# AntreasAntoniou/HowToTrainYourMAMLPytorch

Measured on NVIDIA H100. Metric: meta-tasks/sec (5-way, 5 inner steps, second order), higher is better.
Workload: dtype fp32

## Files before the change

howtotrainyourmamlpytorch_b200/csrc/common.cuh:

```cuda
#pragma once
#include <cuda_runtime.h>
#include <stdint.h>
#include <string>

#define MAML_MAX_LAYERS 4
#define MAML_MAX_STEPS 8
#define BN_EPS_D 1e-5
#define LEAKY_SLOPE_F 0.01f

struct LayerGeom {
  int h, w;
  int cin;
  int gw, G;
  int ph, pw;
  int pgw, pG, pb;
  int guard;
};

struct ConvSrc {
  const float* A; long long a_stride;
  const float* W; long long w_stride;
  int kc;
  int wt;
  int sign;
};

enum { CONV_PLAIN = 0, CONV_FWD_STATS = 1, CONV_TAN_STATS = 2 };

struct ConvArgs {
  ConvSrc src[2]; int nsrc;
  const float* bias; long long bias_stride;
  float* out; long long out_stride;
  int rows;
  int gw, G, h, w;
  int ncols;
  int mode;
  const float* zh; long long zh_stride;
  double* stats; long long stats_stride;
  int tasks;
  double alg_flops;
  int tag;
};

struct Conv0Args {
  const float* X; long long x_stride;
  const float* W; long long w_stride;
  const float* bias; long long bias_stride;
  float* out; long long out_stride;
  int rows, gw, G, h, w, c0, ncols, mode;
  const float* zh; long long zh_stride;
  double* stats; long long stats_stride;
  int tasks;
  double alg_flops;
  int tag;
};

struct WgradArgs {
  const float* A[2]; long long a_stride[2];
  const float* D[2]; long long d_stride[2];
  long long a_plane[2], d_plane[2];
  int nsrc;
  int kc, ncols, rows, gw;
  int rows_per_chunk, nchunks;
  float* partial; long long partial_task_stride; long long chunk_stride;
  int tasks;
  double alg_flops;
  int tag;
};

struct InputGradArgs {
  const float* D[2]; long long d_stride[2];
  const float* W[2]; long long w_stride;
  float* dx; long long dx_stride;
  int nsrc;
  int rows, gw, G, h, w, c0, ncols;
  int tasks;
  double alg_flops;
  int tag;
};

struct BnGeom { int n, h, w, gw, G, ph, pw, pgw, pG, pb, F; };

struct BnActArgs {
  float* z; long long z_stride;
  const double* stats; long long stats_stride;
  const float* gamma; const float* beta;
  float* p; long long p_stride;
  float* p_hi; float* p_lo;
  BnGeom g; int tasks;
  int tag;
};

struct BnActTanArgs {
  float* zdot; long long zdot_stride;
  const float* zdot2;
  const float* zh; long long zh_stride;
  const double* stats_fwd; long long stats_fwd_stride;
  const double* stats_tan; long long stats_tan_stride;
  const float* gamma; const float* beta;
  float* pdot; long long pdot_stride;
  float* pdot_hi; float* pdot_lo;
  BnGeom g; int tasks;
  int tag;
};

struct BnBwdArgs {
  const float* dp; long long dp_stride;
  const float* zh; long long zh_stride;
  const double* stats_fwd; long long stats_fwd_stride;
  double* stats_bwd; long long stats_bwd_stride;
  const float* gamma; const float* beta;
  float* dz; long long dz_stride;
  float* dz_hi; float* dz_lo;
  BnGeom g; int tasks;
  int tag;
};

struct BnBwdTanArgs {
  const float* dp; long long dp_stride;
  const float* dpdot; long long dpdot_stride;
  const float* dpdot2;
  const float* zh; long long zh_stride;
  const float* zhdot; long long zhdot_stride;
  const float* dz; long long dz_stride;
  const double* stats_fwd; long long stats_fwd_stride;
  const double* stats_bwd; long long stats_bwd_stride;
  const double* stats_tan; long long stats_tan_stride;
  double* stats_tbwd; long long stats_tbwd_stride;
  const float* gamma; const float* beta;
  float* dzdot; long long dzdot_stride;
  float* dzdot_hi; float* dzdot_lo;
  BnGeom g; int tasks;
  int tag;
};

struct LnArgs {
  float* z; long long z_stride;
  const float* z2;
  const float* zh; long long zh_stride;
  const float* zhd; long long zhd_stride;
  const float* dp; long long dp_stride;
  const float* dpd; const float* dpd2; long long dpd_stride;
  const float* dz; long long dz_stride;
  float* out; float* out_hi; float* out_lo; long long out_stride;
  const double* st_fwd;
  const double* st_tan;
  const double* st_bwd;
  double* st_out;
// ... 75 lines not shown
void launch_bnbwd_tan(const BnBwdTanArgs& a, cudaStream_t st);
void launch_bnact_ibn(const BnActArgs& a, long long gb_stride, cudaStream_t st);
void launch_bnbwd_ibn(const BnBwdArgs& a, long long gb_stride, cudaStream_t st);
void launch_bnact_tan_ibn(const BnActTanArgs& a, long long gb_stride, const float* gdot, const float* bdot, cudaStream_t st);
void launch_bnbwd_tan_ibn(const BnBwdTanArgs& a, long long gb_stride, const float* gdot, cudaStream_t st);
void launch_ln_stats(const LnArgs& a, bool tan, cudaStream_t st);
void launch_ln_act(const LnArgs& a, bool tan, cudaStream_t st);
void launch_ln_bwd(const LnArgs& a, bool tan, cudaStream_t st);
void launch_ln_bias_grad(const LnArgs& a, bool tan, cudaStream_t st);
bool tail_fusable(const BnGeom& g, int n_rows, int rows_per_cta);
void launch_tail_fused(const BnActArgs& fa, const HeadArgs& ha, const BnBwdArgs& ba, cudaStream_t st);
void launch_tail_tan_fused(const BnActTanArgs& fa, const HeadArgs& ha, const BnBwdTanArgs& ba, cudaStream_t st);
void launch_head(const HeadArgs& a, cudaStream_t st);

void launch_import_theta(const ParamLayout& pl, const float* meta, float* theta0, long long theta_task_stride,
                         int tasks, cudaStream_t st, long long meta_task_stride = 0);
void launch_param_reduce(const ParamLayout& pl, const PartialDesc& pd, const float* partial, int mode,
                         const float* theta_in, float* theta_out, float* g_out, float* tbar,
                         const float* meta, int step, long long task_stride, int tasks, cudaStream_t st,
                         int seg_lo = 0, int seg_hi = -1);
void launch_dots_u(const ParamLayout& pl, float* tbar, const float* tgrad, const float* g, float* u, double* abar,
                   const float* meta, int step, long long task_stride, int tasks, cudaStream_t st);

#define MAML_MAX_RANKS 8
struct CommDev {
  int rank, world;
  float* local_data; long long slot_stride;
  unsigned* local_flags;
  unsigned* seq;
  unsigned* counters;
  const float* peer_data[MAML_MAX_RANKS];
  unsigned* peer_flags[MAML_MAX_RANKS];
  long long* status;
};

struct ExportArgs {
  CommDev comm;
  ParamLayout pl;
  const float* tbar; long long task_stride;
  const double* abar;
  const double* stats; long long stats_task_stride;
  long long st_pass_stride, st_layer_stride;
  const float* losses;
  const float* correct;
  float weights[MAML_MAX_STEPS];
  unsigned target_mask; int num_steps; int training;
  int tasks, task_offset, tasks_global;
  int n_s, n_t;
  int hw[MAML_MAX_LAYERS];
  float* result;
  int per_task; long long result_stride;
  const float* lnb;
  int tag;
};
void launch_export(const ExportArgs& a, cudaStream_t st);
void launch_allreduce(const CommDev& c, float* result, long long n, cudaStream_t st);
void launch_publish(const CommDev& c, const float* src, long long n, cudaStream_t st);

void launch_adam(float* meta, const float* grad, float* m, float* v, long long n, float lr, float bc1, float bc2,
                 const long long* seg_end_host, int nseg, unsigned trainable_mask, unsigned clamp_mask,
                 cudaStream_t st);
void launch_running_update(const float* part_mean, const float* part_var, float* rm, float* rv,
                           const float* decay_dev, int L, int S, int F, cudaStream_t st);
void launch_running_ema_from_stats(const double* stats, long long stats_task_stride, long long layer_stride, int tasks, float* rm,
                                   float* rv, int L, int S, int F, int step, const int* hw_host, int n, cudaStream_t st);

void launch_episode_gather(const float* dataset, const long long* image_index, const int* rot_k, int B, int N, int K, int T, int C,
                           int H, int W, const float* mean, const float* stdv, float* xs, float* xt, long long* ys, long long* yt,
                           cudaStream_t st);

enum { PASS_SUP_FWD = 0, PASS_SUP_BWD = 1, PASS_TGT_FWD = 2, PASS_TGT_BWD = 3, PASS_TAN_FWD = 4, PASS_TAN_BWD = 5,
       PASS_KINDS = 6 };

struct EngineOptions {
  bool no_graph = false;
  bool one_stream = false;
  bool wgrad_tc = true;
  int tc_split = 8;
  int tc_nb = 0;
  bool bn_fuse = true;
  bool tail_fuse = true;
  int tail_onchip = 3;
  int pdl = -1;
  int tc_timeline = -1;
  std::string graph_dot;
};

struct Profiler;
struct LaunchContext {
  const EngineOptions* opt;
  bool pdl;
  cudaStream_t main_stream;
  Profiler* prof;
};
const LaunchContext& launch_ctx();

inline bool pdl_allowed(cudaStream_t st) {
  const LaunchContext& c = launch_ctx();
  return c.pdl && st == c.main_stream;
}
int num_sms();

#define MAML_TRACE_ARMED 0x40000000
static __device__ unsigned long long* t_trace_buf = nullptr;
#define MAML_TRACE_SETTER(fn) void fn(unsigned long long* p) { cudaMemcpyToSymbol(t_trace_buf, &p, sizeof(p)); }
#define MAML_TRACE_CAP 4094
__device__ __forceinline__ void trace_mark(int kid, int tag = 0) {
  if (!(tag & MAML_TRACE_ARMED)) return;
  unsigned long long* t = t_trace_buf;
  if (t != nullptr && threadIdx.x == 0 && blockIdx.x == 0 && blockIdx.y == 0 && blockIdx.z == 0) {
    unsigned long long now;
    asm volatile("mov.u64 %0, %%globaltimer;" : "=l"(now));
    const unsigned long long slot = atomicAdd(t, 1ULL);
    if (slot < MAML_TRACE_CAP) t[1 + slot] = (now << 20) | ((unsigned long long)(tag & 0xfff) << 8) | (unsigned long long)(kid & 0xff);
  }
}
void trace_set_conv(unsigned long long* p);
void trace_set_bn(unsigned long long* p);
void trace_set_head(unsigned long long* p);
void trace_set_param(unsigned long long* p);
void trace_set_tc(unsigned long long* p);

__device__ __forceinline__ void pdl_prologue(int kid = 0, int tag = 0) {
  trace_mark(kid, tag);
  asm volatile("griddepcontrol.launch_dependents;" ::: "memory");
  asm volatile("griddepcontrol.wait;" ::: "memory");
}
__device__ __forceinline__ void pdl_trigger() { asm volatile("griddepcontrol.launch_dependents;" ::: "memory"); }
__device__ __forceinline__ void pdl_wait() { asm volatile("griddepcontrol.wait;" ::: "memory"); }
template <typename... KArgs, typename... Args>
inline void launch_pdl(void (*kernel)(KArgs...), dim3 grid, dim3 block, size_t smem, cudaStream_t st, Args&&... args) {
  cudaLaunchConfig_t cfg{};
  cfg.gridDim = grid; cfg.blockDim = block; cfg.dynamicSmemBytes = smem; cfg.stream = st;
  cudaLaunchAttribute attr[1];
  attr[0].id = cudaLaunchAttributeProgrammaticStreamSerialization;
  attr[0].val.programmaticStreamSerializationAllowed = pdl_allowed(st) ? 1 : 0;
  cfg.attrs = attr; cfg.numAttrs = 1;
  cudaLaunchKernelEx(&cfg, kernel, static_cast<KArgs>(args)...);
}

extern long long g_launch_counter;
extern long long g_launch_base;
extern int g_trace_flag;
inline int launch_tag() { return (int)(g_launch_counter - g_launch_base) | g_trace_flag; }
template <class A> inline A tagged(const A& a) { A t = a; t.tag = launch_tag(); return t; }

#define CUDA_CHECK_LAUNCH() do { g_launch_counter++; } while (0)

enum { PROF_CONV = 0, PROF_CONV0 = 1, PROF_WGRAD = 2, PROF_WGRAD0 = 3, PROF_BN = 4, PROF_HEAD = 5, PROF_PARAM = 6,
       PROF_CATS = 7 };
void prof_begin(Profiler* p, int cat, double flops, cudaStream_t st);
void prof_end(Profiler* p, cudaStream_t st);
struct ProfScope {
  cudaStream_t st; Profiler* prof;
  ProfScope(int cat, double flops, cudaStream_t s) : st(s), prof(launch_ctx().prof) { if (prof) prof_begin(prof, cat, flops, st); }
  ~ProfScope() { if (prof) prof_end(prof, st); }
};
```

howtotrainyourmamlpytorch_b200/csrc/engine.cu:

```cuda
#include <cstdio>
#include <cstdlib>
#include <cstring>
#include <cmath>
#include <string>
#include <vector>

#include "../../include/maml_b200.h"
#include "common.cuh"
#include "tc_common.cuh"

static thread_local std::string g_err;
static int fail(const std::string& m) { g_err = m; return 1; }

#define CK(call) do { cudaError_t e__ = (call); if (e__ != cudaSuccess) { \
  return fail(std::string(#call) + ": " + cudaGetErrorString(e__)); } } while (0)

static inline long long rup(long long x, long long m) { return (x + m - 1) / m * m; }

struct Profiler {
  struct Rec { int cat; double flops; cudaEvent_t a, b; };
  std::vector<Rec> recs;
  std::vector<cudaEvent_t> pool;
  size_t used = 0;
  cudaEvent_t get() {
    if (used == pool.size()) { cudaEvent_t e; cudaEventCreate(&e); pool.push_back(e); }
    return pool[used++];
  }
  void reset() { recs.clear(); used = 0; }
  ~Profiler() { for (auto e : pool) cudaEventDestroy(e); }
};
void prof_begin(Profiler* p, int cat, double flops, cudaStream_t st) {
  Profiler::Rec r; r.cat = cat; r.flops = flops; r.a = p->get(); r.b = p->get();
  cudaEventRecord(r.a, st);
  p->recs.push_back(r);
}
void prof_end(Profiler* p, cudaStream_t st) { cudaEventRecord(p->recs.back().b, st); }

static EngineOptions read_options() {
  auto flag = [](const char* name, bool def) { const char* v = getenv(name); return v ? atoi(v) != 0 : def; };
  auto num = [](const char* name, int def) { const char* v = getenv(name); return v ? atoi(v) : def; };
  auto clamp = [](int v, int lo, int hi) { return std::max(lo, std::min(hi, v)); };
  EngineOptions o;
  o.no_graph = getenv("MAML_B200_NO_GRAPH") != nullptr;
  o.one_stream = getenv("MAML_B200_ONE_STREAM") != nullptr;
  o.wgrad_tc = flag("MAML_B200_WGRAD_TC", o.wgrad_tc);
  o.tc_split = clamp(num("MAML_B200_TC_SPLIT", o.tc_split), 1, 8);
  if (getenv("MAML_B200_TC_NB")) o.tc_nb = clamp(num("MAML_B200_TC_NB", 0), 2, 8);
  o.bn_fuse = flag("MAML_B200_BN_FUSE", o.bn_fuse);
  o.tail_fuse = flag("MAML_B200_TAIL_FUSE", o.tail_fuse);
  o.tail_onchip = num("MAML_B200_TAIL_ONCHIP", o.tail_onchip);
  if (const char* v = getenv("MAML_B200_PDL")) o.pdl = atoi(v) != 0 ? 1 : 0;
  if (getenv("MAML_B200_TC_TIMELINE")) o.tc_timeline = std::max(0, num("MAML_B200_TC_TIMELINE", 0));
  if (const char* v = getenv("MAML_B200_GRAPH_DOT")) o.graph_dot = v;
  return o;
}

struct PassSet {
  int n = 0, slots = 0;
  float* xg = nullptr; long long xg_stride = 0;
  float* ain[MAML_MAX_LAYERS + 1] = {}; long long ain_sz[MAML_MAX_LAYERS + 1] = {};
  float* zh[MAML_MAX_LAYERS] = {}; long long zh_sz[MAML_MAX_LAYERS] = {};
  float* dz[MAML_MAX_LAYERS] = {}; long long dz_sz[MAML_MAX_LAYERS] = {};
  float* dp[MAML_MAX_LAYERS] = {}; long long dp_sz[MAML_MAX_LAYERS] = {};
  float* ain_base[MAML_MAX_LAYERS + 1] = {}; long long ain_plane[MAML_MAX_LAYERS + 1] = {};
  float* dz_base[MAML_MAX_LAYERS] = {}; long long dz_plane[MAML_MAX_LAYERS] = {};
  CUtensorMap ain_map[MAML_MAX_LAYERS][2];
  CUtensorMap dz_map[MAML_MAX_LAYERS][2];
};

struct ChunkPlan { int rows_per_chunk[MAML_MAX_LAYERS]; int nchunks[MAML_MAX_LAYERS]; PartialDesc pd; long long size; int head_groups; };
static inline int head_rows(int n) { return n <= 16 ? 16 : 4; }

struct maml_b200_handle {
  maml_b200_config cfg;
  EngineOptions opt;
  int L, F, N, S, C, H, W, n_s, n_t, maxT, D, pix;
  LayerGeom geo[MAML_MAX_LAYERS];
  ParamLayout pl;
  long long Ppad;
  std::vector<long long> seg_off, seg_size;
  char* ws = nullptr; long long ws_bytes = 0;
  PassSet sup, tgt, tan, tan2;
  float *theta = nullptr, *g = nullptr, *tgrad = nullptr, *tbar = nullptr, *u = nullptr;
  float *sup_partial = nullptr, *tgt_partial = nullptr;
  ChunkPlan plan_sup, plan_tgt;
  double* stats = nullptr; long long stats_task_stride = 0, st_pass_stride = 0, st_layer_stride = 0, stats_count = 0;
  float *losses = nullptr, *correct = nullptr, *decay_dev = nullptr;
  double* abar = nullptr;
  bool ln = false;
  double* ln_stats = nullptr; long long ln_task_stride = 0, ln_pass_stride = 0;
  float* lnb = nullptr;
  long long* zero_labels = nullptr;
  float* pinned = nullptr;
  int pin_slot = 0;
  long long last_launches = 0;
  int last_tasks = 0;
  int fn_kind = 0, fn_tasks = 0, fn_step = 0;
  float* xdot_g = nullptr;
  float* zero_dl = nullptr;
  Profiler prof;
  bool profiling = false;
  cudaStream_t s_cap = nullptr, s_tgt = nullptr, s_tgt2 = nullptr, s_wg = nullptr;
  int tgt_slots = 1;
  cudaEvent_t ev_fork = nullptr, ev_wg = nullptr, ev_pack = nullptr, ev_tgt[MAML_MAX_STEPS] = {};
  cudaEvent_t ev_pre[2 * MAML_MAX_LAYERS] = {};
  bool use_graphs = true;
  bool pdl = false;
  int nb_main = 8;
  bool wg_pending = false;
  struct GraphEntry { maml_b200_iter_args it; const void* p[7]; cudaGraphExec_t exec; long long launches; unsigned long long stamp; };
  std::vector<GraphEntry> graphs;
  unsigned long long graph_clock = 0;
  bool use_tc = false;
  float *pack_theta = nullptr, *pack_u = nullptr;
  long long pack_theta_plane = 0, pack_u_plane = 0, pack_task = 0;
  CUtensorMap theta_map[4], u_map[4];
  CommDev comm{};
  char* comm_block = nullptr; long long comm_bytes = 0;
  void* comm_opened[MAML_MAX_RANKS] = {};
  bool comm_connected = false;
};

enum { FN_NONE = 0, FN_FORWARD = 1, FN_BACKWARD = 2, FN_HVP = 4 };
static void record_call(maml_b200_handle* h, int kind, int n_tasks, int num_step) {
  h->fn_kind = kind; h->fn_tasks = n_tasks; h->fn_step = num_step;
}
static std::string call_names(int kinds) {
  std::string s;
  for (int k : {FN_FORWARD, FN_BACKWARD, FN_HVP})
    if (kinds & k)
      s += std::string(s.empty() ? "" : " or ") + (k == FN_FORWARD ? "maml_b200_net_forward" : k == FN_BACKWARD ? "maml_b200_net_backward" : "maml_b200_net_hvp");
  return s;
}
static int require_call(const maml_b200_handle* h, int kinds, int n_tasks, int num_step, const char* entry) {
// ... 466 lines not shown
  cudaEventRecord(h->ev_wg, h->s_wg);
  h->wg_pending = true;
}

static void reduce_lower(maml_b200_handle* h, const ReduceSpec& rs, const PartialDesc& pd, const float* partial,
                         const float* meta, int T, cudaStream_t st) {
  launch_param_reduce(h->pl, with_bn_sums(h, pd, rs.bn_sums), partial, rs.mode, rs.theta_in, rs.theta_out, rs.g_out, rs.tbar,
                      meta, rs.step, h->Ppad, T, st, 0, seg_per_block(h->pl));
}
static void join_pending(maml_b200_handle* h, cudaStream_t st) {
  if (!h->wg_pending) return;
  cudaStreamWaitEvent(st, h->ev_wg, 0);
  h->wg_pending = false;
}

static void tc_conv(maml_b200_handle* h, int l, int n, const TcOp& op, const float* bias, long long bias_stride,
                    float* out, long long out_stride, int mode, const float* zh, long long zh_stride, double* stats, int T,
                    cudaStream_t st) {
  const LayerGeom& g = h->geo[l];
  TcMaps maps;
  TcConvArgs a{};
  a.kc = h->F; a.rows = n * g.G; a.gw = g.gw; a.G = g.G; a.h = g.h; a.w = g.w; a.ncols = h->F; a.mode = mode; a.tasks = T; a.plan_tasks = h->maxT;
  a.halo = g.gw + 1; a.rpad = tc_conv_rpad(g.gw); a.nb = std::min(tc_conv_ring(h->F, g.gw), h->nb_main);
  a.timeline = (h->opt.tc_timeline == 0 || h->opt.tc_timeline == l) ? 1 : 0;
  maps.m[0] = op.a_maps[0]; maps.m[1] = op.a_maps[1];
  maps.m[2] = op.b_maps[op.b_pair]; maps.m[3] = op.b_maps[op.b_pair + 1];
  a.a_row_base = op.a_row_base; a.a_task_rows = op.a_task_rows; a.sign = op.sign;
  a.b_row_base = op.b_row_base; a.b_task_rows = op.b_task_rows;
  a.bias = bias; a.bias_stride = bias_stride; a.out = out; a.out_stride = out_stride;
  a.zh = zh; a.zh_stride = zh_stride; a.stats = stats; a.stats_stride = h->stats_task_stride;
  a.alg_flops = conv_flops(h, l, n, T, 1);
  launch_conv_tc(maps, a, st);
}

struct FfmaOp { const float* A; long long a_stride; const float* wv; int wt, sign; };

static ConvArgs ffma_conv(const maml_b200_handle* h, int l, int n, int mode, std::initializer_list<FfmaOp> ops,
                          const float* bias_vec, int T) {
  const LayerGeom& g = h->geo[l];
  ConvArgs a{};
  for (const FfmaOp& o : ops) a.src[a.nsrc++] = ConvSrc{o.A, o.a_stride, o.wv + h->pl.w_off[l], h->Ppad, h->F, o.wt, o.sign};
  if (bias_vec) { a.bias = bias_vec + h->pl.b_off[l]; a.bias_stride = h->Ppad; }
  a.rows = n * g.G; a.gw = g.gw; a.G = g.G; a.h = g.h; a.w = g.w; a.ncols = h->F; a.mode = mode;
  if (mode != CONV_PLAIN) a.stats_stride = h->stats_task_stride;
  a.tasks = T;
  a.alg_flops = conv_flops(h, l, n, T, a.nsrc);
  return a;
}

static Conv0Args conv0_args(const maml_b200_handle* h, const PassSet& ps, const float* wv, int mode, int nsrc, int T) {
  const LayerGeom& g = h->geo[0];
  Conv0Args a{};
  a.X = ps.xg; a.x_stride = ps.xg_stride;
  a.W = wv + h->pl.w_off[0]; a.w_stride = h->Ppad;
  a.bias = wv + h->pl.b_off[0]; a.bias_stride = h->Ppad;
  a.rows = ps.n * g.G; a.gw = g.gw; a.G = g.G; a.h = g.h; a.w = g.w; a.c0 = h->C; a.ncols = h->F; a.mode = mode;
  a.stats_stride = h->stats_task_stride; a.tasks = T;
  a.alg_flops = conv_flops(h, 0, ps.n, T, nsrc);
  return a;
}

static WgradArgs wgrad_args(const maml_b200_handle* h, int l, int n, const ChunkPlan& cp, float* partial, int T) {
  const LayerGeom& g = h->geo[l];
  WgradArgs w{};
  w.kc = l == 0 ? h->C : h->F; w.ncols = h->F; w.rows = n * g.G; w.gw = g.gw;
  w.rows_per_chunk = cp.rows_per_chunk[l]; w.nchunks = cp.nchunks[l];
  const int k = seg_per_block(h->pl) * l;
  w.partial = partial + cp.pd.off[k]; w.partial_task_stride = cp.pd.task_stride; w.chunk_stride = cp.pd.cstride[k];
  w.tasks = T;
  return w;
}

struct WgPair { Slot a, d; };

static void launch_wgrad_upper(const maml_b200_handle* h, int l, int n, const ChunkPlan& cp, float* partial, int T,
                               std::initializer_list<WgPair> pairs, cudaStream_t st) {
  const bool tc = h->use_tc && h->opt.wgrad_tc;
  WgradArgs w = wgrad_args(h, l, n, cp, partial, T);
  for (const WgPair& p : pairs) {
    const PassSet& pa = *p.a.ps; const PassSet& pd = *p.d.ps;
    const int k = w.nsrc++;
    w.A[k] = AIN(pa, l, p.a.slot); w.a_stride[k] = STRIDE(pa, ain, l);
    w.D[k] = DZ(pd, l, p.d.slot); w.d_stride[k] = STRIDE(pd, dz, l);
    if (tc) { w.a_plane[k] = pa.ain_plane[l]; w.d_plane[k] = pd.dz_plane[l]; }
  }
  w.alg_flops = conv_flops(h, l, n, T, w.nsrc);
  if (tc) launch_wgrad_tc(w, st);
  else launch_wgrad(w, st);
}

static HeadArgs head_args(const maml_b200_handle* h, int mode, const PassSet& ps, int slot, const float* theta, int T) {
  HeadArgs a{};
  a.mode = mode; a.n = ps.n; a.N = h->N; a.D = h->D; a.scale = 1.f;
  a.f = AIN(ps, h->L, slot); a.f_stride = STRIDE(ps, ain, h->L);
  a.Wfc = theta + h->pl.fcw_off; a.bfc = theta + h->pl.fcb_off; a.theta_stride = h->Ppad;
  a.y = h->zero_labels; a.y_stride = 0;
  a.rows_per_cta = head_rows(ps.n);
  if (mode != HEAD_TARGET_FWD) { a.df = DP(ps, h->L - 1, slot); a.df_stride = STRIDE(ps, dp, h->L - 1); }
  a.tasks = T;
  return a;
}

static void head_grad(const maml_b200_handle* h, HeadArgs& a, float* partial, const ChunkPlan& cp) {
  const int k = seg_per_block(h->pl) * h->L;
  a.gW = partial + cp.pd.off[k]; a.gb = partial + cp.pd.off[k + 1];
  a.g_stride = cp.pd.task_stride; a.g_chunk_stride = cp.pd.cstride[k];
}

static bool support_tail_fused(const maml_b200_handle* h) {
  return h->opt.tail_fuse && !h->ln && !h->pl.inner_bn && tail_fusable(bn_geom(h, h->L - 1, h->n_s), h->n_s, head_rows(h->n_s));
}

enum { CLR_STATS = 1, CLR_ABAR = 2, CLR_LOSSES = 4, CLR_CORRECT = 8, CLR_BWD_STATS = 16 };
static int clear_accumulators(maml_b200_handle* h, unsigned what, cudaStream_t st, int bwd_tasks = 0) {
  if (what & CLR_STATS) CK(cudaMemsetAsync(h->stats, 0, (size_t)h->stats_count * sizeof(double), st));
  if ((what & CLR_STATS) && h->ln) CK(cudaMemsetAsync(h->ln_stats, 0, (size_t)h->ln_task_stride * h->maxT * sizeof(double), st));
  if (what & CLR_BWD_STATS)
    for (int kind : {PASS_TGT_BWD, PASS_TAN_BWD}) {
      CK(cudaMemset2DAsync(h->stats + (long long)kind * MAML_MAX_STEPS * h->st_pass_stride, (size_t)h->stats_task_stride * sizeof(double),
                           0, (size_t)MAML_MAX_STEPS * h->st_pass_stride * sizeof(double), (size_t)bwd_tasks, st));
      if (h->ln)
        CK(cudaMemset2DAsync(h->ln_stats + (long long)kind * h->ln_pass_stride, (size_t)h->ln_task_stride * sizeof(double), 0,
                             (size_t)h->ln_pass_stride * sizeof(double), (size_t)bwd_tasks, st));
    }
  if ((what & (CLR_STATS | CLR_BWD_STATS)) && h->ln) {
    const int tasks = (what & CLR_STATS) ? h->maxT : bwd_tasks;
    CK(cudaMemsetAsync(h->lnb, 0, (size_t)tasks * 2 * h->S * h->pl.lnb_off[h->L] * sizeof(float), st));
  }
  if (what & CLR_ABAR) CK(cudaMemsetAsync(h->abar, 0, (size_t)h->maxT * h->pl.nseg_inner * MAML_MAX_STEPS * sizeof(double), st));
  if (what & CLR_LOSSES) CK(cudaMemsetAsync(h->losses, 0, (size_t)h->maxT * MAML_MAX_STEPS * sizeof(float), st));
  if (what & CLR_CORRECT) CK(cudaMemsetAsync(h->correct, 0, (size_t)h->maxT * sizeof(float), st));
  return 0;
}

static void norm_forward(maml_b200_handle* h, const PassSet& ps, int slot, const float* theta, const float* meta, int l, int step,
                         int stat_kind, int T, cudaStream_t st, BnActArgs* defer_last) {
  if (h->ln) {
    LnArgs a = ln_args(h, l, ps.n, meta, T);
    a.z = ZH(ps, l, slot); a.z_stride = STRIDE(ps, zh, l);
    a.st_fwd = a.st_out = ln_stat_at(h, stat_kind, step, l);
    launch_ln_stats(a, false, st);
    a.out = AIN(ps, l + 1, slot); a.out_stride = STRIDE(ps, ain, l + 1);
    if (h->use_tc && l + 1 < h->L) { a.out_hi = AIN_HI(ps, l + 1, slot); a.out_lo = AIN_LO(ps, l + 1, slot); }
    launch_ln_act(a, false, st);
    return;
  }
  BnActArgs b{};
  b.z = ZH(ps, l, slot); b.z_stride = STRIDE(ps, zh, l);
  b.stats = stat_at(h, stat_kind, step, l); b.stats_stride = h->stats_task_stride;
  const NormParams np = norm_params(h, meta, theta, l, step);
  b.gamma = np.gamma; b.beta = np.beta;
  b.p = AIN(ps, l + 1, slot); b.p_stride = STRIDE(ps, ain, l + 1);
  if (h->use_tc && l + 1 < h->L) { b.p_hi = AIN_HI(ps, l + 1, slot); b.p_lo = AIN_LO(ps, l + 1, slot); }
  b.g = bn_geom(h, l, ps.n); b.tasks = T;
  if (defer_last && l == h->L - 1) *defer_last = b;
  else if (np.stride) launch_bnact_ibn(b, np.stride, st);
  else launch_bnact(b, st);
}

static void norm_backward(maml_b200_handle* h, const PassSet& ps, int slot, const float* theta, const float* meta, int l, int step,
                          int kind_fwd, int kind_bwd, int T, cudaStream_t st, const BnActArgs* fused_act, const HeadArgs* fused_head) {
  if (h->ln) {
    LnArgs a = ln_args(h, l, ps.n, meta, T);
    a.dp = DP(ps, l, slot); a.dp_stride = STRIDE(ps, dp, l);
    a.zh = ZH(ps, l, slot); a.zh_stride = STRIDE(ps, zh, l);
    a.st_fwd = ln_stat_at(h, kind_fwd, step, l); a.st_out = ln_stat_at(h, kind_bwd, step, l);
    a.out = DZ(ps, l, slot); a.out_stride = STRIDE(ps, dz, l);
    if (h->use_tc && l >= 1) { a.out_hi = DZ_HI(ps, l, slot); a.out_lo = DZ_LO(ps, l, slot); }
    launch_ln_bwd(a, false, st);
// ... 921 lines not shown
```

howtotrainyourmamlpytorch_b200/csrc/kernels_tc.cu:

```cuda
#include <cuda.h>
#include <algorithm>
#include <map>
#include <utility>
#include "common.cuh"
#include "tc_common.cuh"

namespace {


__device__ __forceinline__ uint32_t smem_u32(const void* p) { return (uint32_t)__cvta_generic_to_shared(p); }

__device__ __forceinline__ void mbar_init(uint64_t* bar, uint32_t count) {
  asm volatile("mbarrier.init.shared::cta.b64 [%0], %1;" ::"r"(smem_u32(bar)), "r"(count) : "memory");
}
__device__ __forceinline__ void fence_barrier_init() { asm volatile("fence.mbarrier_init.release.cluster;" ::: "memory"); }
__device__ __forceinline__ void mbar_arrive_expect_tx(uint64_t* bar, uint32_t bytes) {
  asm volatile("mbarrier.arrive.expect_tx.shared::cta.b64 _, [%0], %1;" ::"r"(smem_u32(bar)), "r"(bytes) : "memory");
}
__device__ __forceinline__ void mbar_wait(uint64_t* bar, uint32_t parity) {
  const uint32_t addr = smem_u32(bar);
  uint32_t done = 0;
  for (long long spin = 0; spin < (1LL << 26); ++spin) {
    asm volatile("{\n\t.reg .pred p;\n\tmbarrier.try_wait.parity.shared::cta.b64 p, [%1], %2;\n\tselp.u32 %0, 1, 0, p;\n\t}"
                 : "=r"(done) : "r"(addr), "r"(parity) : "memory");
// ... 323 lines not shown
          const float4 v = *reinterpret_cast<const float4*>(trow + c);
          if (owner == zrank) *reinterpret_cast<float4*>(push_local + c) = v;
          else dsmem_st4(push_row + (uint32_t)(c * 4), v);
        }
      }
      if (r == 0) TC_MARK(7);
    }

    int row_lo = 0, row_n = 128;
    const float* sbuf = tile;
    if (nsplit > 1) {
      __syncwarp();
      if (warp >= 4) cluster_wait();
      cluster_sync_all();
      if (threadIdx.x == 0) TC_MARK(10);
      row_n = 128 / nsplit; row_lo = zrank * row_n;
      float* tile2 = reinterpret_cast<float*>(smem + 40 * 1024);
      sbuf = tile2;
      if (warp < 4) {
        const int et = threadIdx.x;
        const float* bias = a.bias ? a.bias + (long long)task * a.bias_stride : nullptr;
        float* outp = a.out + (long long)task * a.out_stride;
        if (nsplit == 2) splitk_reduce<NCOLS, 2>(recv, zrank, et, bias, tile2, outp, j0, a.rows);
        else if (nsplit == 4) splitk_reduce<NCOLS, 4>(recv, zrank, et, bias, tile2, outp, j0, a.rows);
        else splitk_reduce<NCOLS, 8>(recv, zrank, et, bias, tile2, outp, j0, a.rows);
      }
    }

    if (threadIdx.x == 0) TC_MARK(11);
    if (warp < 4) {
      const int et = threadIdx.x;
      const bool want_stats = (a.mode != CONV_PLAIN);
      if (want_stats) {
        asm volatile("bar.sync 2, 128;" ::: "memory");
        constexpr int PARTS = 128 / NCOLS;
        const int col = et % NCOLS, part = et / NCOLS;
        double s1 = 0.0, s2 = 0.0;
        if (part < PARTS) {
          for (int rr = part; rr < row_n; rr += PARTS) {
            if (row_ok[row_lo + rr]) {
              const float v = sbuf[rr * P4 + col];
              if (a.mode == CONV_FWD_STATS) { s1 += (double)v; s2 += (double)v * (double)v; }
              else { s1 += (double)v; s2 += (double)zbuf[rr * P4 + col] * (double)v; }
            }
          }
          if (part < 2) { sred[part][col][0] = s1; sred[part][col][1] = s2; }
        }
        if (PARTS > 2) {
          asm volatile("bar.sync 2, 128;" ::: "memory");
          if (part >= 2 && part < PARTS) { atomicAdd(&sred[part & 1][col][0], s1); atomicAdd(&sred[part & 1][col][1], s2); }
        }
        asm volatile("bar.sync 2, 128;" ::: "memory");
        if (et < NCOLS * 2) {
          const int c = et >> 1, which = et & 1;
          double* stats = a.stats + (long long)task * a.stats_stride;
          atomicAdd(&stats[c * 2 + which], sred[0][c][which] + sred[1][c][which]);
        }
      }
    }
    if (threadIdx.x == 0) TC_MARK(12);
    if (threadIdx.x == 0) TC_MARK(8);
  }
  trace_mark(22 | 0x80, a.tag);
}

template <int NC>
__device__ __forceinline__ void wgmma_tf32_rs(float (&d)[NC / 2], const uint32_t (&a)[4], uint64_t bdesc) {
  if constexpr (NC == 16) wgmma_tf32_rs_n16(d, a, bdesc);
  else if constexpr (NC == 32) wgmma_tf32_rs_n32(d, a, bdesc);
  else if constexpr (NC == 48) wgmma_tf32_rs_n48(d, a, bdesc);
  else wgmma_tf32_rs_n64(d, a, bdesc);
}

__device__ __forceinline__ void cp_async16(uint32_t dst, const void* src, bool ok) {
  asm volatile("cp.async.cg.shared.global [%0], [%1], 16, %2;" ::"r"(dst), "l"(src), "r"(ok ? 16 : 0) : "memory");
}
__device__ __forceinline__ void cp_async_arrive(uint64_t* bar) {
  asm volatile("cp.async.mbarrier.arrive.noinc.shared::cta.b64 [%0];" ::"r"(smem_u32(bar)) : "memory");
}

constexpr int WG_NS = 3;
constexpr int WG_THREADS = 384;

template <int NC> struct WgSlot {
  static constexpr int BT = NC * 128;
  static constexpr int AP = NC + 8;
  static constexpr int AW = 34 * AP * 4;
  static constexpr int DW = 32 * NC * 4;
  static constexpr int A_OFF = 2 * BT, D_OFF = A_OFF + 2 * AW, DF_OFF = D_OFF + 2 * DW;
  static constexpr int BYTES = (DF_OFF + DW + 1023) / 1024 * 1024;
};
template <int NC> constexpr size_t wgrad_tc_smem() { return (size_t)WG_NS * WgSlot<NC>::BYTES + 1024; }

template <int NC>
__global__ void __launch_bounds__(WG_THREADS, 1) wgrad_tc_row_kernel(const WgradArgs a) {
  pdl_prologue(27, a.tag);
  using S = WgSlot<NC>;
  constexpr int R = NC / 2;
  constexpr int Q = NC / 4;
  extern __shared__ uint8_t smem_raw[];
  uint8_t* smem = reinterpret_cast<uint8_t*>((reinterpret_cast<uintptr_t>(smem_raw) + 1023) & ~(uintptr_t)1023);
  __shared__ uint64_t full[WG_NS];
  const int task = blockIdx.y;
  const int chunk = blockIdx.x / 3, ky = blockIdx.x - chunk * 3;
  const int sh0 = (ky - 1) * a.gw - 1;
  const int r_begin = chunk * a.rows_per_chunk;
  const int r_end = min(a.rows, r_begin + a.rows_per_chunk);
  const int guard = a.gw + 2;
  const int steps = r_end > r_begin ? (r_end - r_begin + 31) / 32 : 0;
  const int nit = steps * a.nsrc;
  const bool bias_cta = (ky == 1);
  const int tid = threadIdx.x, warp = tid >> 5, lane = tid & 31;

  if (tid == 0) {
    for (int s = 0; s < WG_NS; ++s) mbar_init(&full[s], WG_THREADS);
    fence_barrier_init();
  }
  __syncthreads();

  auto load_stage = [&](int it) {
    const int slot = it % WG_NS;
    const int s = it / steps;
    const int r0 = r_begin + (it - s * steps) * 32;
    const float* Ah = a.A[s] + (long long)task * a.a_stride[s] + a.a_plane[s];
    const float* Al = Ah + a.a_plane[s];
    const float* Df = a.D[s] + (long long)task * a.d_stride[s];
    const float* Dh = Df + a.d_plane[s];
    const float* Dl = Dh + a.d_plane[s];
    const uint32_t base = smem_u32(smem + (size_t)slot * S::BYTES);
    for (int e = tid; e < 34 * Q; e += WG_THREADS) {
      const int r = e / Q, c4 = e - r * Q;
      const int jr = r0 + sh0 + r;
      const bool ok = jr >= -guard && jr < a.rows + guard;
      const long long go = ok ? (long long)jr * NC + c4 * 4 : 0;
      const uint32_t so = (uint32_t)((r * S::AP + c4 * 4) * 4);
      cp_async16(base + S::A_OFF + so, Ah + go, ok);
      cp_async16(base + S::A_OFF + S::AW + so, Al + go, ok);
    }
    const bool want_f = bias_cta && s == 0;
    for (int e = tid; e < 32 * Q; e += WG_THREADS) {
      const int r = e / Q;
      const int jr = r0 + r;
      const bool ok = jr < r_end;
      const long long go = ok ? (long long)jr * NC + (e - r * Q) * 4 : 0;
      cp_async16(base + S::D_OFF + e * 16, Dh + go, ok);
      cp_async16(base + S::D_OFF + S::DW + e * 16, Dl + go, ok);
      if (want_f) cp_async16(base + S::DF_OFF + e * 16, Df + go, ok);
    }
    cp_async_arrive(&full[slot]);
  };

  const int kx = warp >> 2;
  const int c0 = 16 * (warp & 3) + (lane >> 2), t4 = lane & 3;
  const bool c_ok = c0 < NC;
  float big[R], small[R], tot[R];
#pragma unroll
  for (int i = 0; i < R; ++i) { big[i] = 0.f; small[i] = 0.f; tot[i] = 0.f; }
  float bacc = 0.f;

  auto transpose = [&](int it) {
    const int slot = it % WG_NS;
    uint8_t* sb = smem + (size_t)slot * S::BYTES;
    mbar_wait(&full[slot], (uint32_t)(it / WG_NS) & 1u);
    for (int e = tid; e < 2 * 8 * NC; e += WG_THREADS) {
      const int pl = e / (8 * NC), rem = e - pl * 8 * NC;
      const int j4 = rem / NC, f = rem - j4 * NC;
      const float* src = reinterpret_cast<const float*>(sb + S::D_OFF + pl * S::DW) + (4 * j4) * NC + f;
      const float4 v = make_float4(src[0], src[NC], src[2 * NC], src[3 * NC]);
      *reinterpret_cast<float4*>(sb + pl * S::BT + f * 128 + ((j4 ^ (f & 7)) << 4)) = v;
    }
    if (bias_cta && tid < NC && it < steps) {
      const float* df = reinterpret_cast<const float*>(sb + S::DF_OFF) + tid;
#pragma unroll 8
      for (int r = 0; r < 32; ++r) bacc += df[r * NC];
    }
    asm volatile("fence.proxy.async.shared::cta;" ::: "memory");
  };

  for (int i = 0; i < WG_NS - 1 && i < nit; ++i) load_stage(i);
  if (nit > 0) transpose(0);
  for (int it = 0; it < nit; ++it) {
    const uint8_t* sb = smem + (size_t)(it % WG_NS) * S::BYTES;
    __syncthreads();
    if (it + WG_NS - 1 < nit) load_stage(it + WG_NS - 1);
    const float* wh = reinterpret_cast<const float*>(sb + S::A_OFF) + (kx + t4) * S::AP + c0;
    const float* wl = wh + S::AW / 4;
    uint32_t ah[4][4], al[4][4];
#pragma unroll
    for (int k = 0; k < 4; ++k)
#pragma unroll
      for (int q = 0; q < 4; ++q) {
        const int o = (8 * k + ((q & 2) ? 4 : 0)) * S::AP + ((q & 1) ? 8 : 0);
        ah[k][q] = c_ok ? __float_as_uint(wh[o]) : 0u;
        al[k][q] = c_ok ? __float_as_uint(wl[o]) : 0u;
      }
    const uint64_t desc_h = make_desc_sw128(smem_u32(sb)), desc_l = desc_h + (uint64_t)(S::BT >> 4);
    wgmma_fence();
#pragma unroll
    for (int k = 0; k < 4; ++k) {
      wgmma_tf32_rs<NC>(big, ah[k], desc_h + 2 * k);
      wgmma_tf32_rs<NC>(small, ah[k], desc_l + 2 * k);
      wgmma_tf32_rs<NC>(small, al[k], desc_h + 2 * k);
    }
    wgmma_commit();
    if (it + 1 < nit) transpose(it + 1);
    wgmma_wait<0>();
    reg_fence<R>(big);
    reg_fence<R>(small);
#pragma unroll
    for (int i = 0; i < R; ++i) { tot[i] += big[i] + small[i]; big[i] = 0.f; small[i] = 0.f; }
    reg_fence<R>(big);
    reg_fence<R>(small);
  }

  float* P = a.partial + (long long)task * a.partial_task_stride + (long long)a.chunk_stride * chunk;
  const int tap = ky * 3 + kx;
#pragma unroll
  for (int i = 0; i < NC / 8; ++i)
#pragma unroll
    for (int hh = 0; hh < 2; ++hh) {
      const int c = c0 + 8 * hh;
      if (c < NC)
        *reinterpret_cast<float2*>(P + (long long)(tap * NC + c) * NC + 8 * i + 2 * t4) = make_float2(tot[4 * i + 2 * hh], tot[4 * i + 2 * hh + 1]);
    }
  if (bias_cta && tid < NC) P[(long long)9 * NC * NC + tid] = bacc;
}


}

int tc_read_timeline(long long* out16) { return cudaMemcpyFromSymbol(out16, g_tc_timeline, 16 * sizeof(long long)) == cudaSuccess ? 0 : 1; }

void launch_wgrad_tc(const WgradArgs& a, cudaStream_t st) {
  ProfScope prof_scope__(PROF_WGRAD, a.alg_flops, st);
  dim3 grid(a.nchunks * 3, a.tasks);
  if (a.ncols == 64) launch_pdl(wgrad_tc_row_kernel<64>, grid, dim3(WG_THREADS), wgrad_tc_smem<64>(), st, tagged(a));
  else if (a.ncols == 48) launch_pdl(wgrad_tc_row_kernel<48>, grid, dim3(WG_THREADS), wgrad_tc_smem<48>(), st, tagged(a));
  else if (a.ncols == 32) launch_pdl(wgrad_tc_row_kernel<32>, grid, dim3(WG_THREADS), wgrad_tc_smem<32>(), st, tagged(a));
  else launch_pdl(wgrad_tc_row_kernel<16>, grid, dim3(WG_THREADS), wgrad_tc_smem<16>(), st, tagged(a));
  CUDA_CHECK_LAUNCH();
}

int tc_conv_rpad(int gw) { return ((128 + 2 * (gw + 1)) + 7) / 8 * 8; }
int tc_conv_ring(int ncols, int gw, size_t extra) {
  const long long avail = 227LL * 1024 - 4096  - 1024  - 4LL * tc_conv_rpad(gw) * 128 - (long long)extra;
  long long nb = avail / (2LL * ncols * 128);
  if (nb > 8) nb = 8;
  return (int)nb;
}
size_t tc_conv_extra_bytes(int ncols, int S, bool tangent) {
  const size_t row = (size_t)(ncols + 4) * 4;
  return (S > 1 ? 128 * row : 0) + (tangent ? (size_t)(128 / S) * row : 0);
}
static size_t tc_conv_smem_for(int ncols, int gw, int nb) { return (size_t)4 * tc_conv_rpad(gw) * 128 + (size_t)nb * 2 * ncols * 128 + 1024; }

int tc_conv_prepare() {
  const int maxs = 227 * 1024 - 4096;
  cudaError_t e1 = cudaFuncSetAttribute(conv_tc_kernel<64>, cudaFuncAttributeMaxDynamicSharedMemorySize, maxs);
  cudaError_t e2 = cudaFuncSetAttribute(conv_tc_kernel<32>, cudaFuncAttributeMaxDynamicSharedMemorySize, maxs);
  cudaError_t e3 = cudaFuncSetAttribute(conv_tc_kernel<48>, cudaFuncAttributeMaxDynamicSharedMemorySize, maxs);
  cudaError_t e4 = cudaFuncSetAttribute(conv_tc_kernel<16>, cudaFuncAttributeMaxDynamicSharedMemorySize, maxs);
  cudaError_t w1 = cudaFuncSetAttribute(wgrad_tc_row_kernel<64>, cudaFuncAttributeMaxDynamicSharedMemorySize, (int)wgrad_tc_smem<64>());
  cudaError_t w2 = cudaFuncSetAttribute(wgrad_tc_row_kernel<48>, cudaFuncAttributeMaxDynamicSharedMemorySize, (int)wgrad_tc_smem<48>());
  cudaError_t w3 = cudaFuncSetAttribute(wgrad_tc_row_kernel<32>, cudaFuncAttributeMaxDynamicSharedMemorySize, (int)wgrad_tc_smem<32>());
  cudaError_t w4 = cudaFuncSetAttribute(wgrad_tc_row_kernel<16>, cudaFuncAttributeMaxDynamicSharedMemorySize, (int)wgrad_tc_smem<16>());
  return (e1 == cudaSuccess && e2 == cudaSuccess && e3 == cudaSuccess && e4 == cudaSuccess && w1 == cudaSuccess &&
          w2 == cudaSuccess && w3 == cudaSuccess && w4 == cudaSuccess) ? 0 : 1;
}

template <int NCOLS>
static int max_clusters(size_t smem, int S) {
  static std::map<std::pair<size_t, int>, int> cache;
  auto it = cache.find({smem, S});
  if (it != cache.end()) return it->second;
  cudaLaunchConfig_t cfg{};
  cfg.gridDim = dim3(1, 1, S); cfg.blockDim = dim3(TC_THREADS); cfg.dynamicSmemBytes = smem;
  cudaLaunchAttribute attr[1];
  attr[0].id = cudaLaunchAttributeClusterDimension;
  attr[0].val.clusterDim.x = 1; attr[0].val.clusterDim.y = 1; attr[0].val.clusterDim.z = S;
  cfg.attrs = attr; cfg.numAttrs = 1;
  int n = 0;
  if (cudaOccupancyMaxActiveClusters(&n, conv_tc_kernel<NCOLS>, &cfg) != cudaSuccess) { cudaGetLastError(); n = 0; }
  cache[{smem, S}] = n;
  return n;
}

template <int NCOLS>
static void launch_conv_tc_n(const TcMaps& maps, const TcConvArgs& a_in, cudaStream_t st) {
  TcConvArgs a = a_in;
  const int tiles = ((a.rows + 127) / 128) * (a.plan_tasks > a.tasks ? a.plan_tasks : a.tasks);
  const int stages = ((a.kc + 31) / 32) * 9;
  const size_t recv_bytes = tc_conv_extra_bytes(NCOLS, 2, false);
  const size_t split_smem = tc_conv_smem_for(NCOLS, a.gw, std::min(a.nb, tc_conv_ring(NCOLS, a.gw, recv_bytes))) + recv_bytes;
  int S = 1;
  for (int cand = launch_ctx().opt->tc_split; cand >= 2; cand >>= 1) {
    if (cand > 8 || stages < 2 * cand) continue;
    if (tiles <= max_clusters<NCOLS>(split_smem, cand)) { S = cand; break; }
  }
  dim3 grid((a.rows + 127) / 128, a.tasks, S);
  const size_t extra = tc_conv_extra_bytes(NCOLS, S, a.mode == CONV_TAN_STATS);
  a.nb = std::min(a.nb, tc_conv_ring(NCOLS, a.gw, extra));
  const size_t smem = tc_conv_smem_for(NCOLS, a.gw, a.nb) + extra;
  if (S == 1) {
    launch_pdl(conv_tc_kernel<NCOLS>, grid, dim3(TC_THREADS), smem, st, maps, tagged(a));
    return;
  }
  cudaLaunchConfig_t cfg{};
  cfg.gridDim = grid; cfg.blockDim = dim3(TC_THREADS); cfg.dynamicSmemBytes = smem; cfg.stream = st;
  cudaLaunchAttribute attr[1];
  attr[0].id = cudaLaunchAttributeClusterDimension;
  attr[0].val.clusterDim.x = 1; attr[0].val.clusterDim.y = 1; attr[0].val.clusterDim.z = S;
  cfg.attrs = attr; cfg.numAttrs = 1;
  cudaLaunchKernelEx(&cfg, conv_tc_kernel<NCOLS>, maps, tagged(a));
}

void launch_conv_tc(const TcMaps& maps, const TcConvArgs& a, cudaStream_t st) {
  ProfScope prof_scope__(PROF_CONV, a.alg_flops, st);
  if (a.ncols == 64) launch_conv_tc_n<64>(maps, a, st);
  else if (a.ncols == 48) launch_conv_tc_n<48>(maps, a, st);
  else if (a.ncols == 32) launch_conv_tc_n<32>(maps, a, st);
  else launch_conv_tc_n<16>(maps, a, st);
  CUDA_CHECK_LAUNCH();
}

__device__ __forceinline__ float tf32_rna(float x) {
  uint32_t r;
  asm("cvt.rna.tf32.f32 %0, %1;" : "=r"(r) : "f"(x));
  return __uint_as_float(r);
}

__global__ void __launch_bounds__(256) pack_weights_kernel(ParamLayout pl, const float* __restrict__ theta,
                                                           long long theta_task_stride, float* __restrict__ pack,
                                                           long long pack_task_stride, long long plane_stride, int tag) {
  pdl_prologue(21, tag);
  __shared__ float s_hi[64 * 65], s_lo[64 * 65];
  const int F = pl.F, FF = F * F, task = blockIdx.y;
  const int l = 1 + blockIdx.x / 9, tap = blockIdx.x % 9;
  const long long tile = (long long)tap * FF;
  const float* src = theta + (long long)task * theta_task_stride + pl.w_off[l] + tile;
  float* p = pack + (long long)task * pack_task_stride + (long long)(l - 1) * 9 * FF + tile;
  for (int i = threadIdx.x; i < FF; i += blockDim.x) {
    const int c = i / F, f = i - c * F;
    const float x = src[i];
    const float hi = tf32_rna(x), lo = tf32_rna(x - hi);
    p[i] = hi;
    p[plane_stride + i] = lo;
    s_hi[f * (F + 1) + c] = hi;
    s_lo[f * (F + 1) + c] = lo;
  }
  __syncthreads();
  for (int i = threadIdx.x; i < FF; i += blockDim.x) {
    const int f = i / F, c = i - f * F;
    p[2 * plane_stride + i] = s_hi[f * (F + 1) + c];
    p[3 * plane_stride + i] = s_lo[f * (F + 1) + c];
  }
}

void launch_pack_weights(const ParamLayout& pl, const float* theta, long long theta_task_stride, float* pack,
                         long long pack_task_stride, long long plane_stride, int tasks, cudaStream_t st) {
  ProfScope prof_scope__(PROF_PARAM, 0.0, st);
  if (pl.L <= 1) return;
  dim3 grid(9 * (pl.L - 1), tasks);
  launch_pdl(pack_weights_kernel, dim3(grid), dim3(256), (size_t)(0), st, pl, theta, theta_task_stride, pack, pack_task_stride, plane_stride, launch_tag());
  CUDA_CHECK_LAUNCH();
}

MAML_TRACE_SETTER(trace_set_tc)
```

Measured before the change: 2691.

## Split fp32 to tf32 hi/lo in-kernel for wgrad and add persistent work loop

The wgrad tensor-core kernel now loads the full fp32 activations and output gradients once and splits them into tf32 hi/lo parts on chip, instead of reading precomputed hi/lo planes from global memory. This reduces global traffic and shared memory per pipeline stage, so the separate fp32 copy for the bias sum is no longer needed. It also turns the grid into a flat work list with an optional persistent mode, where the CTA count is set by an environment variable and the load pipeline carries across work items. The cost is extra conversion instructions in the transpose and fragment-load paths. Writers that produce the hi/lo planes may now do unneeded work.

```diff
diff --git a/howtotrainyourmamlpytorch_b200/csrc/common.cuh b/howtotrainyourmamlpytorch_b200/csrc/common.cuh
--- a/howtotrainyourmamlpytorch_b200/csrc/common.cuh
+++ b/howtotrainyourmamlpytorch_b200/csrc/common.cuh
@@ -58,12 +58,12 @@
 struct WgradArgs {
   const float* A[2]; long long a_stride[2];
   const float* D[2]; long long d_stride[2];
-  long long a_plane[2], d_plane[2];
   int nsrc;
   int kc, ncols, rows, gw;
   int rows_per_chunk, nchunks;
   float* partial; long long partial_task_stride; long long chunk_stride;
   int tasks;
+  int ctas;
   double alg_flops;
   int tag;
 };
@@ -305,6 +305,7 @@
   bool tail_fuse = true;
   int tail_onchip = 3;
   int pdl = -1;
+  int wgrad_ctas = 0;
   int tc_timeline = -1;
   std::string graph_dot;
 };
diff --git a/howtotrainyourmamlpytorch_b200/csrc/engine.cu b/howtotrainyourmamlpytorch_b200/csrc/engine.cu
--- a/howtotrainyourmamlpytorch_b200/csrc/engine.cu
+++ b/howtotrainyourmamlpytorch_b200/csrc/engine.cu
@@ -50,6 +50,7 @@
   o.tail_fuse = flag("MAML_B200_TAIL_FUSE", o.tail_fuse);
   o.tail_onchip = num("MAML_B200_TAIL_ONCHIP", o.tail_onchip);
   if (const char* v = getenv("MAML_B200_PDL")) o.pdl = atoi(v) != 0 ? 1 : 0;
+  o.wgrad_ctas = std::max(0, num("MAML_B200_WGRAD_CTAS", o.wgrad_ctas));
   if (getenv("MAML_B200_TC_TIMELINE")) o.tc_timeline = std::max(0, num("MAML_B200_TC_TIMELINE", 0));
   if (const char* v = getenv("MAML_B200_GRAPH_DOT")) o.graph_dot = v;
   return o;
@@ -682,9 +683,9 @@
     const int k = w.nsrc++;
     w.A[k] = AIN(pa, l, p.a.slot); w.a_stride[k] = STRIDE(pa, ain, l);
     w.D[k] = DZ(pd, l, p.d.slot); w.d_stride[k] = STRIDE(pd, dz, l);
-    if (tc) { w.a_plane[k] = pa.ain_plane[l]; w.d_plane[k] = pd.dz_plane[l]; }
   }
   w.alg_flops = conv_flops(h, l, n, T, w.nsrc);
+  w.ctas = h->opt.wgrad_ctas;
   if (tc) launch_wgrad_tc(w, st);
   else launch_wgrad(w, st);
 }
diff --git a/howtotrainyourmamlpytorch_b200/csrc/kernels_tc.cu b/howtotrainyourmamlpytorch_b200/csrc/kernels_tc.cu
--- a/howtotrainyourmamlpytorch_b200/csrc/kernels_tc.cu
+++ b/howtotrainyourmamlpytorch_b200/csrc/kernels_tc.cu
@@ -429,15 +429,35 @@
 constexpr int WG_NS = 3;
 constexpr int WG_THREADS = 384;
 
+__device__ __forceinline__ float tf32_rna(float x) {
+  uint32_t r;
+  asm("cvt.rna.tf32.f32 %0, %1;" : "=r"(r) : "f"(x));
+  return __uint_as_float(r);
+}
+
 template <int NC> struct WgSlot {
   static constexpr int BT = NC * 128;
   static constexpr int AP = NC + 8;
   static constexpr int AW = 34 * AP * 4;
   static constexpr int DW = 32 * NC * 4;
-  static constexpr int A_OFF = 2 * BT, D_OFF = A_OFF + 2 * AW, DF_OFF = D_OFF + 2 * DW;
-  static constexpr int BYTES = (DF_OFF + DW + 1023) / 1024 * 1024;
+  static constexpr int A_OFF = 2 * BT, D_OFF = A_OFF + AW;
+  static constexpr int BYTES = (D_OFF + DW + 1023) / 1024 * 1024;
 };
 template <int NC> constexpr size_t wgrad_tc_smem() { return (size_t)WG_NS * WgSlot<NC>::BYTES + 1024; }
+
+struct WgItem {
+  int chunk, ky, task, r_begin, r_end, steps, nit;
+  __device__ WgItem(const WgradArgs& a, int w) {
+    const int per_task = a.nchunks * 3;
+    task = w / per_task;
+    const int x = w - task * per_task;
+    chunk = x / 3; ky = x - chunk * 3;
+    r_begin = chunk * a.rows_per_chunk;
+    r_end = min(a.rows, r_begin + a.rows_per_chunk);
+    steps = r_end > r_begin ? (r_end - r_begin + 31) / 32 : 0;
+    nit = steps * a.nsrc;
+  }
+};
 
 template <int NC>
 __global__ void __launch_bounds__(WG_THREADS, 1) wgrad_tc_row_kernel(const WgradArgs a) {
@@ -448,15 +468,8 @@
   extern __shared__ uint8_t smem_raw[];
   uint8_t* smem = reinterpret_cast<uint8_t*>((reinterpret_cast<uintptr_t>(smem_raw) + 1023) & ~(uintptr_t)1023);
   __shared__ uint64_t full[WG_NS];
-  const int task = blockIdx.y;
-  const int chunk = blockIdx.x / 3, ky = blockIdx.x - chunk * 3;
-  const int sh0 = (ky - 1) * a.gw - 1;
-  const int r_begin = chunk * a.rows_per_chunk;
-  const int r_end = min(a.rows, r_begin + a.rows_per_chunk);
+  const int nwork = a.nchunks * 3 * a.tasks;
   const int guard = a.gw + 2;
-  const int steps = r_end > r_begin ? (r_end - r_begin + 31) / 32 : 0;
-  const int nit = steps * a.nsrc;
-  const bool bias_cta = (ky == 1);
   const int tid = threadIdx.x, warp = tid >> 5, lane = tid & 31;
 
   if (tid == 0) {
@@ -465,36 +478,38 @@
   }
   __syncthreads();
 
-  auto load_stage = [&](int it) {
-    const int slot = it % WG_NS;
-    const int s = it / steps;
-    const int r0 = r_begin + (it - s * steps) * 32;
-    const float* Ah = a.A[s] + (long long)task * a.a_stride[s] + a.a_plane[s];
-    const float* Al = Ah + a.a_plane[s];
-    const float* Df = a.D[s] + (long long)task * a.d_stride[s];
-    const float* Dh = Df + a.d_plane[s];
-    const float* Dl = Dh + a.d_plane[s];
+  int ld_w = blockIdx.x, ld_it = 0, ld_g = 0;
+  WgItem ld(a, ld_w);
+  auto ld_skip_done = [&]() {
+    while (ld_w < nwork && ld_it >= ld.nit) { ld_w += gridDim.x; ld_it = 0; if (ld_w < nwork) ld = WgItem(a, ld_w); }
+  };
+  ld_skip_done();
+  auto load_next = [&]() {
+    if (ld_w >= nwork) return;
+    const int slot = ld_g % WG_NS;
+    const int s = ld_it / ld.steps;
+    const int r0 = ld.r_begin + (ld_it - s * ld.steps) * 32;
+    const int sh0 = (ld.ky - 1) * a.gw - 1;
+    const float* Af = a.A[s] + (long long)ld.task * a.a_stride[s];
+    const float* Df = a.D[s] + (long long)ld.task * a.d_stride[s];
     const uint32_t base = smem_u32(smem + (size_t)slot * S::BYTES);
     for (int e = tid; e < 34 * Q; e += WG_THREADS) {
       const int r = e / Q, c4 = e - r * Q;
       const int jr = r0 + sh0 + r;
       const bool ok = jr >= -guard && jr < a.rows + guard;
       const long long go = ok ? (long long)jr * NC + c4 * 4 : 0;
-      const uint32_t so = (uint32_t)((r * S::AP + c4 * 4) * 4);
-      cp_async16(base + S::A_OFF + so, Ah + go, ok);
-      cp_async16(base + S::A_OFF + S::AW + so, Al + go, ok);
-    }
-    const bool want_f = bias_cta && s == 0;
+      cp_async16(base + S::A_OFF + (uint32_t)((r * S::AP + c4 * 4) * 4), Af + go, ok);
+    }
     for (int e = tid; e < 32 * Q; e += WG_THREADS) {
       const int r = e / Q;
       const int jr = r0 + r;
-      const bool ok = jr < r_end;
+      const bool ok = jr < ld.r_end;
       const long long go = ok ? (long long)jr * NC + (e - r * Q) * 4 : 0;
-      cp_async16(base + S::D_OFF + e * 16, Dh + go, ok);
-      cp_async16(base + S::D_OFF + S::DW + e * 16, Dl + go, ok);
-      if (want_f) cp_async16(base + S::DF_OFF + e * 16, Df + go, ok);
+      cp_async16(base + S::D_OFF + e * 16, Df + go, ok);
     }
     cp_async_arrive(&full[slot]);
+    ++ld_g; ++ld_it;
+    ld_skip_done();
   };
 
   const int kx = warp >> 2;
@@ -502,75 +517,86 @@
   const bool c_ok = c0 < NC;
   float big[R], small[R], tot[R];
 #pragma unroll
-  for (int i = 0; i < R; ++i) { big[i] = 0.f; small[i] = 0.f; tot[i] = 0.f; }
-  float bacc = 0.f;
-
-  auto transpose = [&](int it) {
-    const int slot = it % WG_NS;
+  for (int i = 0; i < R; ++i) { big[i] = 0.f; small[i] = 0.f; }
+
+  auto transpose = [&](int g) {
+    const int slot = g % WG_NS;
     uint8_t* sb = smem + (size_t)slot * S::BYTES;
-    mbar_wait(&full[slot], (uint32_t)(it / WG_NS) & 1u);
-    for (int e = tid; e < 2 * 8 * NC; e += WG_THREADS) {
-      const int pl = e / (8 * NC), rem = e - pl * 8 * NC;
-      const int j4 = rem / NC, f = rem - j4 * NC;
-      const float* src = reinterpret_cast<const float*>(sb + S::D_OFF + pl * S::DW) + (4 * j4) * NC + f;
+    mbar_wait(&full[slot], (uint32_t)(g / WG_NS) & 1u);
+    for (int e = tid; e < 8 * NC; e += WG_THREADS) {
+      const int j4 = e / NC, f = e - j4 * NC;
+      const float* src = reinterpret_cast<const float*>(sb + S::D_OFF) + (4 * j4) * NC + f;
       const float4 v = make_float4(src[0], src[NC], src[2 * NC], src[3 * NC]);
-      *reinterpret_cast<float4*>(sb + pl * S::BT + f * 128 + ((j4 ^ (f & 7)) << 4)) = v;
-    }
-    if (bias_cta && tid < NC && it < steps) {
-      const float* df = reinterpret_cast<const float*>(sb + S::DF_OFF) + tid;
-#pragma unroll 8
-      for (int r = 0; r < 32; ++r) bacc += df[r * NC];
+      const float4 h = make_float4(tf32_rna(v.x), tf32_rna(v.y), tf32_rna(v.z), tf32_rna(v.w));
+      const float4 l = make_float4(tf32_rna(v.x - h.x), tf32_rna(v.y - h.y), tf32_rna(v.z - h.z), tf32_rna(v.w - h.w));
+      const int off = f * 128 + ((j4 ^ (f & 7)) << 4);
+      *reinterpret_cast<float4*>(sb + off) = h;
+      *reinterpret_cast<float4*>(sb + S::BT + off) = l;
     }
     asm volatile("fence.proxy.async.shared::cta;" ::: "memory");
   };
 
-  for (int i = 0; i < WG_NS - 1 && i < nit; ++i) load_stage(i);
-  if (nit > 0) transpose(0);
-  for (int it = 0; it < nit; ++it) {
-    const uint8_t* sb = smem + (size_t)(it % WG_NS) * S::BYTES;
-    __syncthreads();
-    if (it + WG_NS - 1 < nit) load_stage(it + WG_NS - 1);
-    const float* wh = reinterpret_cast<const float*>(sb + S::A_OFF) + (kx + t4) * S::AP + c0;
-    const float* wl = wh + S::AW / 4;
-    uint32_t ah[4][4], al[4][4];
-#pragma unroll
-    for (int k = 0; k < 4; ++k)
-#pragma unroll
-      for (int q = 0; q < 4; ++q) {
-        const int o = (8 * k + ((q & 2) ? 4 : 0)) * S::AP + ((q & 1) ? 8 : 0);
-        ah[k][q] = c_ok ? __float_as_uint(wh[o]) : 0u;
-        al[k][q] = c_ok ? __float_as_uint(wl[o]) : 0u;
-      }
-    const uint64_t desc_h = make_desc_sw128(smem_u32(sb)), desc_l = desc_h + (uint64_t)(S::BT >> 4);
-    wgmma_fence();
-#pragma unroll
-    for (int k = 0; k < 4; ++k) {
-      wgmma_tf32_rs<NC>(big, ah[k], desc_h + 2 * k);
-      wgmma_tf32_rs<NC>(small, ah[k], desc_l + 2 * k);
-      wgmma_tf32_rs<NC>(small, al[k], desc_h + 2 * k);
-    }
-    wgmma_commit();
-    if (it + 1 < nit) transpose(it + 1);
-    wgmma_wait<0>();
-    reg_fence<R>(big);
-    reg_fence<R>(small);
-#pragma unroll
-    for (int i = 0; i < R; ++i) { tot[i] += big[i] + small[i]; big[i] = 0.f; small[i] = 0.f; }
-    reg_fence<R>(big);
-    reg_fence<R>(small);
-  }
-
-  float* P = a.partial + (long long)task * a.partial_task_stride + (long long)a.chunk_stride * chunk;
-  const int tap = ky * 3 + kx;
-#pragma unroll
-  for (int i = 0; i < NC / 8; ++i)
-#pragma unroll
-    for (int hh = 0; hh < 2; ++hh) {
-      const int c = c0 + 8 * hh;
-      if (c < NC)
-        *reinterpret_cast<float2*>(P + (long long)(tap * NC + c) * NC + 8 * i + 2 * t4) = make_float2(tot[4 * i + 2 * hh], tot[4 * i + 2 * hh + 1]);
-    }
-  if (bias_cta && tid < NC) P[(long long)9 * NC * NC + tid] = bacc;
+  for (int i = 0; i < WG_NS - 1; ++i) load_next();
+  int g = 0;
+  if (ld_g > 0) transpose(0);
+  for (int w = blockIdx.x; w < nwork; w += gridDim.x) {
+    const WgItem I(a, w);
+    const bool bias_cta = (I.ky == 1);
+#pragma unroll
+    for (int i = 0; i < R; ++i) tot[i] = 0.f;
+    float bacc = 0.f;
+    for (int it = 0; it < I.nit; ++it, ++g) {
+      const uint8_t* sb = smem + (size_t)(g % WG_NS) * S::BYTES;
+      __syncthreads();
+      load_next();
+      const float* wf = reinterpret_cast<const float*>(sb + S::A_OFF) + (kx + t4) * S::AP + c0;
+      uint32_t ah[4][4], al[4][4];
+#pragma unroll
+      for (int k = 0; k < 4; ++k)
+#pragma unroll
+        for (int q = 0; q < 4; ++q) {
+          const int o = (8 * k + ((q & 2) ? 4 : 0)) * S::AP + ((q & 1) ? 8 : 0);
+          const float x = c_ok ? wf[o] : 0.f;
+          const float hi = tf32_rna(x);
+          ah[k][q] = __float_as_uint(hi);
+          al[k][q] = __float_as_uint(tf32_rna(x - hi));
+        }
+      const uint64_t desc_h = make_desc_sw128(smem_u32(sb)), desc_l = desc_h + (uint64_t)(S::BT >> 4);
+      wgmma_fence();
+#pragma unroll
+      for (int k = 0; k < 4; ++k) {
+        wgmma_tf32_rs<NC>(big, ah[k], desc_h + 2 * k);
+        wgmma_tf32_rs<NC>(small, ah[k], desc_l + 2 * k);
+        wgmma_tf32_rs<NC>(small, al[k], desc_h + 2 * k);
+      }
+      wgmma_commit();
+      if (bias_cta && tid < NC && it < I.steps) {
+        const float* df = reinterpret_cast<const float*>(sb + S::D_OFF) + tid;
+#pragma unroll 8
+        for (int r = 0; r < 32; ++r) bacc += df[r * NC];
+      }
+      if (g + 1 < ld_g) transpose(g + 1);
+      wgmma_wait<0>();
+      reg_fence<R>(big);
+      reg_fence<R>(small);
+#pragma unroll
+      for (int i = 0; i < R; ++i) { tot[i] += big[i] + small[i]; big[i] = 0.f; small[i] = 0.f; }
+      reg_fence<R>(big);
+      reg_fence<R>(small);
+    }
+
+    float* P = a.partial + (long long)I.task * a.partial_task_stride + (long long)a.chunk_stride * I.chunk;
+    const int tap = I.ky * 3 + kx;
+#pragma unroll
+    for (int i = 0; i < NC / 8; ++i)
+#pragma unroll
+      for (int hh = 0; hh < 2; ++hh) {
+        const int c = c0 + 8 * hh;
+        if (c < NC)
+          *reinterpret_cast<float2*>(P + (long long)(tap * NC + c) * NC + 8 * i + 2 * t4) = make_float2(tot[4 * i + 2 * hh], tot[4 * i + 2 * hh + 1]);
+      }
+    if (bias_cta && tid < NC) P[(long long)9 * NC * NC + tid] = bacc;
+  }
 }
 
 
@@ -580,7 +606,8 @@
 
 void launch_wgrad_tc(const WgradArgs& a, cudaStream_t st) {
   ProfScope prof_scope__(PROF_WGRAD, a.alg_flops, st);
-  dim3 grid(a.nchunks * 3, a.tasks);
+  const int items = a.nchunks * 3 * a.tasks;
+  dim3 grid(a.ctas > 0 ? std::min(a.ctas, items) : items);
   if (a.ncols == 64) launch_pdl(wgrad_tc_row_kernel<64>, grid, dim3(WG_THREADS), wgrad_tc_smem<64>(), st, tagged(a));
   else if (a.ncols == 48) launch_pdl(wgrad_tc_row_kernel<48>, grid, dim3(WG_THREADS), wgrad_tc_smem<48>(), st, tagged(a));
   else if (a.ncols == 32) launch_pdl(wgrad_tc_row_kernel<32>, grid, dim3(WG_THREADS), wgrad_tc_smem<32>(), st, tagged(a));
@@ -668,12 +695,6 @@
   else if (a.ncols == 32) launch_conv_tc_n<32>(maps, a, st);
   else launch_conv_tc_n<16>(maps, a, st);
   CUDA_CHECK_LAUNCH();
-}
-
-__device__ __forceinline__ float tf32_rna(float x) {
-  uint32_t r;
-  asm("cvt.rna.tf32.f32 %0, %1;" : "=r"(r) : "f"(x));
-  return __uint_as_float(r);
 }
 
 __global__ void __launch_bounds__(256) pack_weights_kernel(ParamLayout pl, const float* __restrict__ theta,
```

Result: no change. 2700, median of 6 (+0.3%).
